# jkulhanek/tetra-nerf

Measured on NVIDIA H100. Metric: rays/sec (4096-ray batch, 300k-tet mesh), higher is better.
Workload: dtype f32 (trace/interp/compositing) + f16w2 tensor-core MLP (fp16 activations x fp16 hi/lo weights, f32 accumulate; per-sample density/colour within 1e-4 of the fp32 oracle, tests/test_gpu_render.py)

## Files before the change

tetra-nerf_b200/csrc/tn_mlp.cuh:

```cuda
#pragma once
#include "tn_common.cuh"
#include "tn_tc.cuh"

namespace tn {

#ifndef TN_MLP_WGS
#define TN_MLP_WGS 3
#endif
constexpr uint32_t MLP_WGS = TN_MLP_WGS;
constexpr uint32_t MLP_THREADS = 128 * MLP_WGS;
constexpr uint32_t MLP_TILE = 64;
constexpr uint32_t MLP_W_BYTES = 32768 + 3 * 65536;
constexpr uint32_t MLP_W_COARSE = 32768 + 2 * 65536;
constexpr uint32_t MLP_OFF_HEAD = MLP_W_BYTES;
constexpr uint32_t MLP_OFF_BARS = MLP_OFF_HEAD + 520 * 4;
constexpr uint32_t MLP_SMEM_BYTES = MLP_OFF_BARS + 8 + 8 * MLP_WGS;
static_assert(MLP_SMEM_BYTES <= 232448, "k_mlp shared memory exceeds 227 KB");
__host__ __device__ constexpr uint32_t mlp_off_layer(int l) { return l == 0 ? 0u : 32768u + 65536u * (uint32_t)(l - 1); }

struct MlpParams {
    const uint32_t *n_active;
    uint32_t S;
    const uint4 *vi;
    const float *bary;
    const float *fshadow;
    const uint8_t *wimg;
    const float *bias;
    const float *head;
    const float *dirbias;
    float *out;
    uint32_t *tile_ctr;
};

constexpr uint32_t MLP_NO_TILE = 0xFFFFFFFFu;

__device__ __forceinline__ float softplus_f(float x) { return x > 20.0f ? x : log1pf(expf(x)); }
__device__ __forceinline__ float sigmoid_f(float x) { return 1.0f / (1.0f + expf(-x)); }

__device__ __forceinline__ float2 ldg_stream2(const float *p) {
    float2 v;
    asm volatile("ld.global.nc.L1::no_allocate.v2.f32 {%0, %1}, [%2];" : "=f"(v.x), "=f"(v.y) : "l"(p));
    return v;
}
__device__ __forceinline__ float4 ldg_stream(const float4 *p) {
    float4 v;
    asm volatile("ld.global.nc.L1::no_allocate.v4.f32 {%0, %1, %2, %3}, [%4];" : "=f"(v.x), "=f"(v.y), "=f"(v.z), "=f"(v.w) : "l"(p));
    return v;
}

__device__ __forceinline__ void wg_sync(uint32_t wg) { asm volatile("bar.sync %0, 128;" ::"r"(1u + wg) : "memory"); }

template <int PREC>
__device__ __forceinline__ void to_operand(float e0, float e1, uint32_t &hi, uint32_t &lo) {
    if (PREC == 2) hi = tc::pack2_f16(e0, e1);
    else tc::split_pack2(e0, e1, hi, lo);
}

template <int PREC>
__device__ __forceinline__ void gather_rows(const uint4 *__restrict__ vi, const float *__restrict__ bary, const float *__restrict__ fshadow, uint64_t row0,
                                            uint64_t total_rows, uint32_t t, uint32_t (&xh)[16], uint32_t (&xl)[16]) {
#pragma unroll
    for (int rr = 0; rr < 2; ++rr) {
        const uint64_t row = row0 + 8u * rr;
        uint4 v = make_uint4(TN_EMPTY, TN_EMPTY, TN_EMPTY, TN_EMPTY);
        float b0 = 0.f, b1 = 0.f, b2 = 0.f;
        if (row < total_rows) {
            v = __ldg(vi + row);
            b0 = __ldg(bary + 3 * row); b1 = __ldg(bary + 3 * row + 1); b2 = __ldg(bary + 3 * row + 2);
        }
        const bool m = v.x != TN_EMPTY;
        const float w0 = __fsub_rn(1.0f, __fadd_rn(__fadd_rn(b0, b1), b2));
        const float *f0 = fshadow + (size_t)v.x * 64 + 2 * t, *f1 = fshadow + (size_t)v.y * 64 + 2 * t;
        const float *f2 = fshadow + (size_t)v.z * 64 + 2 * t, *f3 = fshadow + (size_t)v.w * 64 + 2 * t;
#pragma unroll
        for (int c = 0; c < 8; ++c) {
            float2 o = make_float2(0.f, 0.f);
            if (m) {
                const float2 a0 = ldg_stream2(f0 + 8 * c), a1 = ldg_stream2(f1 + 8 * c), a2 = ldg_stream2(f2 + 8 * c), a3 = ldg_stream2(f3 + 8 * c);
                o.x = __fmaf_rn(b0, a1.x, 0.f); o.y = __fmaf_rn(b0, a1.y, 0.f);
                o.x = __fmaf_rn(b1, a2.x, o.x); o.y = __fmaf_rn(b1, a2.y, o.y);
                o.x = __fmaf_rn(b2, a3.x, o.x); o.y = __fmaf_rn(b2, a3.y, o.y);
                o.x = __fmaf_rn(w0, a0.x, o.x); o.y = __fmaf_rn(w0, a0.y, o.y);
            }
            const int i = 4 * (c >> 1) + 2 * (c & 1) + rr;
            to_operand<PREC>(o.x, o.y, xh[i], xl[i]);
        }
    }
}

template <int PREC, int KSTEPS>
__device__ __forceinline__ void layer_mma(float (&d)[64], const uint32_t (&ah)[4 * KSTEPS], const uint32_t (&al)[4 * KSTEPS], uint32_t w) {
    using namespace tc;
    wgmma_fence();
#pragma unroll
    for (int kk = 0; kk < KSTEPS; ++kk) {
        const uint32_t wb = w + (uint32_t)(kk >> 2) * 32768u + (uint32_t)(kk & 3) * 32u;
        const uint32_t a[4] = {ah[4 * kk], ah[4 * kk + 1], ah[4 * kk + 2], ah[4 * kk + 3]};
        if (PREC == 2) {
            wgmma_rs_f16_n128<0>(d, a, make_desc(wb), kk > 0 ? 1u : 0u);
            wgmma_rs_f16_n128<0>(d, a, make_desc(wb + 16384u), 1u);
        } else {
            const uint32_t b[4] = {al[4 * kk], al[4 * kk + 1], al[4 * kk + 2], al[4 * kk + 3]};
            wgmma_rs_bf16_n128<0>(d, a, make_desc(wb), kk > 0 ? 1u : 0u);
            wgmma_rs_bf16_n128<0>(d, b, make_desc(wb), 1u);
            wgmma_rs_bf16_n128<0>(d, a, make_desc(wb + 16384u), 1u);
        }
    }
    wgmma_commit();
    wgmma_wait0();
    reg_fence(d);
}

template <bool FINE, int PREC>
__global__ void __launch_bounds__(MLP_THREADS, 1) k_mlp(const MlpParams p) {
    using namespace tc;
    extern __shared__ __align__(1024) uint8_t tn_mlp_smem[];
    uint8_t *smem = tn_mlp_smem;
    const float *head_s = reinterpret_cast<const float *>(smem + MLP_OFF_HEAD);
    uint64_t *w_bar = reinterpret_cast<uint64_t *>(smem + MLP_OFF_BARS);
    volatile uint32_t *slots = reinterpret_cast<volatile uint32_t *>(smem + MLP_OFF_BARS + 8);

    constexpr int L = FINE ? 4 : 3;
    constexpr uint32_t WBYTES = FINE ? MLP_W_BYTES : MLP_W_COARSE;
    const uint32_t wg = threadIdx.x >> 7, tid = threadIdx.x & 127u;
    const uint32_t warp = tid >> 5, lane = threadIdx.x & 31u, g = lane >> 2, t = lane & 3u;
    const uint32_t n_active = *p.n_active;
    const uint64_t total_rows = (uint64_t)n_active * p.S;
    const uint32_t ntiles = (uint32_t)((total_rows + MLP_TILE - 1) / MLP_TILE);
    if (blockIdx.x * MLP_WGS >= ntiles) return;

    if (threadIdx.x == 0) {
        mbar_init(w_bar, 1);
        fence_barrier_init();
    }
    for (uint32_t i = threadIdx.x; i < 516; i += MLP_THREADS) const_cast<float *>(head_s)[i] = p.head[i];
    if (tid == 0) {
        const uint32_t first = blockIdx.x * MLP_WGS + wg;
        slots[2 * wg] = first < ntiles ? first : MLP_NO_TILE;
    }
    __syncthreads();
    if (threadIdx.x == 0) {
        mbar_arrive_expect_tx(w_bar, WBYTES);
        for (uint32_t off = 0; off < WBYTES; off += 16384) tma_bulk_g2s(smem + off, p.wimg + off, 16384, w_bar);
    }
    const uint32_t wsm = smem_u32(smem);
    const float *wd = head_s, *wc = head_s + 128;
    bool weights_ready = false;

#pragma unroll 1
    for (uint32_t n = 0;; ++n) {
        wg_sync(wg);
        const uint32_t tile = slots[2 * wg + (n & 1u)];
        if (tile == MLP_NO_TILE) break;
        if (tid == 0) {
            const uint32_t nx = gridDim.x * MLP_WGS + atomicAdd(p.tile_ctr, 1u);
            slots[2 * wg + ((n + 1u) & 1u)] = nx < ntiles ? nx : MLP_NO_TILE;
        }
        const uint64_t row0 = (uint64_t)tile * MLP_TILE + warp * 16u + g, row1 = row0 + 8u;

        uint32_t ah[32], al[32];
        {
            uint32_t xh[16], xl[16];
            gather_rows<PREC>(p.vi, p.bary, p.fshadow, row0, total_rows, t, xh, xl);
            if (!weights_ready) { mbar_wait(w_bar, 0); weights_ready = true; }
            float d[64];
            layer_mma<PREC, 4>(d, xh, xl, wsm + mlp_off_layer(0));
#pragma unroll
            for (int j = 0; j < 16; ++j) {
                const float2 b = __ldg(reinterpret_cast<const float2 *>(p.bias + 8 * j + 2 * t));
                const int i = 4 * (j >> 1) + 2 * (j & 1);
                to_operand<PREC>(fmaxf(d[4 * j] + b.x, 0.f), fmaxf(d[4 * j + 1] + b.y, 0.f), ah[i], al[i]);
                to_operand<PREC>(fmaxf(d[4 * j + 2] + b.x, 0.f), fmaxf(d[4 * j + 3] + b.y, 0.f), ah[i + 1], al[i + 1]);
            }
        }
        float dens0 = 0.f, dens1 = 0.f;
#pragma unroll
        for (int l = 1; l < 3; ++l) {
            float d[64];
            layer_mma<PREC, 8>(d, ah, al, wsm + mlp_off_layer(l));
            const float *bias = p.bias + 128 * l;
#pragma unroll
            for (int j = 0; j < 16; ++j) {
                const int c = 8 * j + 2 * (int)t;
                const float2 b = __ldg(reinterpret_cast<const float2 *>(bias + c));
                const float x0 = fmaxf(d[4 * j] + b.x, 0.f), x1 = fmaxf(d[4 * j + 1] + b.y, 0.f);
                const float y0 = fmaxf(d[4 * j + 2] + b.x, 0.f), y1 = fmaxf(d[4 * j + 3] + b.y, 0.f);
                if (l == 2) {
                    dens0 = fmaf(x0, wd[c], dens0); dens0 = fmaf(x1, wd[c + 1], dens0);
                    dens1 = fmaf(y0, wd[c], dens1); dens1 = fmaf(y1, wd[c + 1], dens1);
                }
                if (l < L - 1) {
                    const int i = 4 * (j >> 1) + 2 * (j & 1);
                    to_operand<PREC>(x0, x1, ah[i], al[i]);
                    to_operand<PREC>(y0, y1, ah[i + 1], al[i + 1]);
                }
            }
        }
        float col0[3] = {0.f, 0.f, 0.f}, col1[3] = {0.f, 0.f, 0.f};
        if (FINE) {
            float d[64];
            layer_mma<PREC, 8>(d, ah, al, wsm + mlp_off_layer(3));
            const float *db0 = p.dirbias + (size_t)((uint32_t)min(row0, total_rows - 1) / p.S) * 128;
            const float *db1 = p.dirbias + (size_t)((uint32_t)min(row1, total_rows - 1) / p.S) * 128;
#pragma unroll
            for (int j = 0; j < 16; ++j) {
                const int c = 8 * j + 2 * (int)t;
                const float2 b0 = __ldg(reinterpret_cast<const float2 *>(db0 + c)), b1 = __ldg(reinterpret_cast<const float2 *>(db1 + c));
                const float x0 = fmaxf(d[4 * j] + b0.x, 0.f), x1 = fmaxf(d[4 * j + 1] + b0.y, 0.f);
                const float y0 = fmaxf(d[4 * j + 2] + b1.x, 0.f), y1 = fmaxf(d[4 * j + 3] + b1.y, 0.f);
#pragma unroll
                for (int ch = 0; ch < 3; ++ch) {
                    const float *w = wc + 128 * ch;
                    col0[ch] = fmaf(x1, w[c + 1], fmaf(x0, w[c], col0[ch]));
                    col1[ch] = fmaf(y1, w[c + 1], fmaf(y0, w[c], col1[ch]));
                }
            }
        }
#pragma unroll
        for (int s = 1; s <= 2; s <<= 1) {
            dens0 += __shfl_xor_sync(0xffffffffu, dens0, s);
            dens1 += __shfl_xor_sync(0xffffffffu, dens1, s);
            if (FINE) {
#pragma unroll
                for (int ch = 0; ch < 3; ++ch) {
                    col0[ch] += __shfl_xor_sync(0xffffffffu, col0[ch], s);
                    col1[ch] += __shfl_xor_sync(0xffffffffu, col1[ch], s);
                }
            }
        }
        if (t < 2) {
            const uint64_t row = t == 0 ? row0 : row1;
            const float dn = t == 0 ? dens0 : dens1;
            if (row < total_rows) {
                const float sigma = softplus_f(dn + head_s[512]);
                if (FINE) {
                    const float c0 = t == 0 ? col0[0] : col1[0], c1 = t == 0 ? col0[1] : col1[1], c2 = t == 0 ? col0[2] : col1[2];
                    reinterpret_cast<float4 *>(p.out)[row] =
                        make_float4(sigma, sigmoid_f(c0 + head_s[513]), sigmoid_f(c1 + head_s[514]), sigmoid_f(c2 + head_s[515]));
                } else {
                    p.out[row] = sigma;
                }
            }
        }
    }
    if (!weights_ready) mbar_wait(w_bar, 0);
}

}
```

tetra-nerf_b200/csrc/tn_mlp_bwd.cuh:

```cuda
#pragma once
#include <type_traits>

#include "tn_common.cuh"
#include "tn_mlp.cuh"
#include "tn_tc.cuh"

namespace tn {

constexpr uint32_t BWD_THREADS = 128;
constexpr uint32_t BWD_TILE = 64;
constexpr uint32_t BWD_STAGE = 32768;
constexpr uint32_t BWD_OFF_RING = 0;
constexpr uint32_t BWD_OFF_X = 65536;
constexpr uint32_t BWD_OFF_H = 81920;
constexpr uint32_t BWD_OFF_DA = BWD_OFF_H + 3 * 32768;
constexpr uint32_t BWD_OFF_HEAD = BWD_OFF_DA + 32768;
constexpr uint32_t BWD_OFF_SUMS = BWD_OFF_HEAD + 2048;
constexpr uint32_t BWD_OFF_BARS = BWD_OFF_SUMS + 7 * 512;
constexpr uint32_t BWD_SMEM_BYTES = BWD_OFF_BARS + 32;
static_assert(BWD_SMEM_BYTES <= 232448, "k_mlp_bwd shared memory exceeds 227 KB");
static_assert(BWD_OFF_X % 1024 == 0 && BWD_OFF_H % 1024 == 0 && BWD_OFF_DA % 1024 == 0, "swizzled operands need 1024-byte alignment");
constexpr uint32_t BWD_WIMG_BYTES = 7 * BWD_STAGE;
constexpr uint32_t BWD_NSEQ = 14;

struct MlpBwdParams {
    const uint32_t *n_active;
    uint32_t S;
    const uint4 *vi;
    const float *bary;
    const float *fshadow;
    const uint8_t *wimg;
    const float *bias;
    const float *head;
    const float *dirbias;
    const float4 *dout;
    float *gshadow;
    float *gw;
    float *g_dirbias;
    uint32_t *tile_ctr;
};
struct MlpBwdDetParams : MlpBwdParams {
    float *part;
    float *gdb_part;
    float *dx;
};
template <bool DET>
using MlpBwdParamsT = typename std::conditional<DET, MlpBwdDetParams, MlpBwdParams>::type;
constexpr uint32_t GW_W1 = 0, GW_W2 = 8192, GW_W3 = 24576, GW_W4B = 40960, GW_B1 = 57344, GW_B2 = 57472, GW_B3 = 57600, GW_WD = 57728, GW_WC = 57856,
                   GW_SUMS = 58240 , GW_W4DIR = 58244 , GW_B4 = 61700, GW_TOTAL = 61828;

constexpr uint32_t BWD_PARTS = 256;
constexpr uint32_t BWD_PART_STRIDE = GW_SUMS;
constexpr uint32_t BWD_DET_OFF_BARS = BWD_OFF_SUMS + 4 * 7 * 512;
constexpr uint32_t BWD_DET_SMEM_BYTES = BWD_DET_OFF_BARS + 32;
static_assert(BWD_DET_SMEM_BYTES <= 232448, "k_mlp_bwd<true> shared memory exceeds 227 KB");
__host__ __device__ __forceinline__ uint32_t bwd_part_lo(uint32_t q, uint32_t ntiles) { return (uint32_t)(((uint64_t)q * ntiles) / BWD_PARTS); }
__host__ __device__ __forceinline__ uint32_t bwd_part_of(uint32_t tile, uint32_t ntiles) {
    return (uint32_t)((((uint64_t)tile + 1) * BWD_PARTS - 1) / ntiles);
}
__device__ __forceinline__ uint32_t bwd_det_first(uint32_t q, uint32_t step, uint32_t ntiles) {
    for (; q < BWD_PARTS; q += step)
        if (bwd_part_lo(q, ntiles) < bwd_part_lo(q + 1, ntiles)) return bwd_part_lo(q, ntiles);
    return MLP_NO_TILE;
}

__device__ __forceinline__ void red_add_v2(float *dst, float a, float b) {
    asm volatile("red.global.add.v2.f32 [%0], {%1, %2};" ::"l"(dst), "f"(a), "f"(b) : "memory");
}
__device__ __forceinline__ void red_add_v4(float *dst, float a, float b, float c, float d) {
    asm volatile("red.global.add.v4.f32 [%0], {%1, %2, %3, %4};" ::"l"(dst), "f"(a), "f"(b), "f"(c), "f"(d) : "memory");
}
__device__ __forceinline__ float4 quad_of_row(float2 p0, float2 p1, uint32_t t) {
    const bool odd = (t & 1u) != 0u;
    const float2 send = odd ? p0 : p1;
    float2 recv;
    recv.x = __shfl_xor_sync(0xffffffffu, send.x, 1);
    recv.y = __shfl_xor_sync(0xffffffffu, send.y, 1);
    return odd ? make_float4(recv.x, recv.y, p1.x, p1.y) : make_float4(p0.x, p0.y, recv.x, recv.y);
}

__device__ __forceinline__ void st_pair(uint32_t base, uint32_t R, uint32_t j, uint32_t t, uint32_t lo_off, uint32_t h, uint32_t l) {
    const uint32_t rowoff = (R >> 3) * 1024u + (R & 7u) * 128u + 4u * t;
    asm volatile(
        "{\n\t.reg .b32 a, x, y;\n\t"
        "and.b32 x, %2, 7;\n\txor.b32 x, x, %3;\n\tshl.b32 x, x, 4;\n\t"
        "shr.b32 y, %2, 3;\n\tshl.b32 y, y, 13;\n\t"
        "add.u32 a, %0, %1;\n\tadd.u32 a, a, x;\n\tadd.u32 a, a, y;\n\t"
        "st.shared.b32 [a], %5;\n\tadd.u32 a, a, %4;\n\tst.shared.b32 [a], %6;\n\t}" ::"r"(base),
        "r"(rowoff), "r"(j), "r"(R & 7u), "r"(lo_off), "r"(h), "r"(l)
        : "memory");
}

template <bool DET = false>
__device__ __forceinline__ void colsum2(float *dst, uint32_t c, float s0, float s1, uint32_t lane, uint32_t warp = 0) {
#pragma unroll
    for (int m = 4; m <= 16; m <<= 1) {
        s0 += __shfl_xor_sync(0xffffffffu, s0, m);
        s1 += __shfl_xor_sync(0xffffffffu, s1, m);
    }
    if constexpr (DET) {
        if (lane < 4) { float *w = dst + warp * (7u * 128u); w[c] += s0; w[c + 1] += s1; }
    } else {
        if (lane < 4) { atomicAdd(dst + c, s0); atomicAdd(dst + c + 1, s1); }
    }
}

template <int NB, bool DET = false>
__device__ __forceinline__ void dw_half(uint32_t sDA, uint32_t sHb, uint32_t h_lo_off, uint32_t mh, float *dst, uint32_t warp, uint32_t g, uint32_t t,
                                        bool first = false) {
    using namespace tc;
    float d[32 * NB];
#pragma unroll
    for (int i = 0; i < 32 * NB; ++i) d[i] = 0.f;
    wgmma_fence();
#pragma unroll
    for (int term = 0; term < 3; ++term) {
        const uint32_t ao = term == 1 ? 16384u : 0u, bo = term == 2 ? h_lo_off : 0u;
#pragma unroll
        for (uint32_t kk = 0; kk < 4; ++kk) {
            const uint64_t da = make_desc(sDA + ao + mh * 8192u + kk * 2048u, 8192u, 1024u);
            const uint64_t db = make_desc(sHb + bo + kk * 2048u, 8192u, 1024u);
            if constexpr (NB == 2) wgmma_ss_bf16_n128<1, 1>(d, da, db, 1u);
            else wgmma_ss_bf16_n64<1, 1>(d, da, db, 1u);
        }
    }
    wgmma_commit();
    wgmma_wait0();
    reg_fence(d);
    const uint32_t o = mh * 64u + warp * 16u + g + 8u * (t & 1u);
#pragma unroll
    for (int j = 0; j < 4 * NB * 2; ++j) {
        const float4 q = quad_of_row(make_float2(d[4 * j], d[4 * j + 1]), make_float2(d[4 * j + 2], d[4 * j + 3]), t);
        if constexpr (DET) {
            float4 *a = reinterpret_cast<float4 *>(dst + (size_t)o * (64u * NB) + 8u * j + 4u * (t >> 1));
            float4 r = q;
            if (!first) { const float4 b = *a; r = make_float4(b.x + q.x, b.y + q.y, b.z + q.z, b.w + q.w); }
            *a = r;
        } else {
            red_add_v4(dst + (size_t)o * (64u * NB) + 8u * j + 4u * (t >> 1), q.x, q.y, q.z, q.w);
        }
    }
}

template <int N>
__device__ __forceinline__ void zero(float (&d)[N]) {
#pragma unroll
    for (int i = 0; i < N; ++i) d[i] = 0.f;
}

__device__ __forceinline__ void frag_pair(float x0, float x1, float y0, float y1, int j, uint32_t (&ah)[32], uint32_t (&al)[32]) {
    const int i = 4 * (j >> 1) + 2 * (j & 1);
    tc::split_pack2(x0, x1, ah[i], al[i]);
    tc::split_pack2(y0, y1, ah[i + 1], al[i + 1]);
}

template <bool DET>
__global__ void __launch_bounds__(BWD_THREADS, 1) k_mlp_bwd(const MlpBwdParamsT<DET> p) {
    using namespace tc;
    extern __shared__ __align__(1024) uint8_t tn_bwd_smem[];
    constexpr uint32_t OFF_BARS = DET ? BWD_DET_OFF_BARS : BWD_OFF_BARS;
    uint8_t *smem = tn_bwd_smem;
    float *head_s = reinterpret_cast<float *>(smem + BWD_OFF_HEAD);
    float *sums = reinterpret_cast<float *>(smem + BWD_OFF_SUMS);
    uint64_t *ring_full = reinterpret_cast<uint64_t *>(smem + OFF_BARS);
    volatile uint32_t *slots = reinterpret_cast<volatile uint32_t *>(smem + OFF_BARS + 16);

    const uint32_t tid = threadIdx.x, warp = tid >> 5, lane = tid & 31u, g = lane >> 2, t = lane & 3u;
    const uint32_t n_active = *p.n_active;
    const uint64_t total_rows = (uint64_t)n_active * p.S;
    const uint32_t ntiles = (uint32_t)((total_rows + BWD_TILE - 1) / BWD_TILE);
    uint32_t first_tile = blockIdx.x;
    if constexpr (DET) {
        if (ntiles == 0) return;
        first_tile = bwd_det_first(blockIdx.x, gridDim.x, ntiles);
        if (first_tile == MLP_NO_TILE) return;
    } else {
        if (blockIdx.x >= ntiles) return;
    }

    if (tid == 0) {
        mbar_init(&ring_full[0], 1); mbar_init(&ring_full[1], 1);
        fence_barrier_init();
        slots[0] = first_tile;
    }
    for (uint32_t i = tid; i < 512; i += BWD_THREADS) head_s[i] = p.head[i];
    for (uint32_t i = tid; i < (DET ? 4u : 1u) * 7 * 128; i += BWD_THREADS) sums[i] = 0.f;
    __syncthreads();
    const uint32_t sR = smem_u32(smem + BWD_OFF_RING), sX = smem_u32(smem + BWD_OFF_X), sH = smem_u32(smem + BWD_OFF_H), sDA = smem_u32(smem + BWD_OFF_DA);
    const float *wd = head_s, *wc = head_s + 128;

    auto ring_issue = [&](uint32_t i) {
        const uint32_t q = i % BWD_NSEQ;
        const uint32_t img = q < 7u ? q : (q == 13u ? 0u : (q & 1u ? 12u - q : 14u - q));
        uint64_t *bar = &ring_full[i & 1u];
        mbar_arrive_expect_tx(bar, BWD_STAGE);
        tma_bulk_g2s(smem + BWD_OFF_RING + (i & 1u) * BWD_STAGE, p.wimg + img * BWD_STAGE, 16384, bar);
        tma_bulk_g2s(smem + BWD_OFF_RING + (i & 1u) * BWD_STAGE + 16384u, p.wimg + img * BWD_STAGE + 16384u, 16384, bar);
    };
    if (tid == 0) ring_issue(0);
    uint32_t seq = 0;
    auto ring_acquire = [&](bool more) -> uint32_t {
        wg_sync(0);
        if (tid == 0 && more) ring_issue(seq + 1u);
        mbar_wait(&ring_full[seq & 1u], (seq >> 1) & 1u);
        const uint32_t w = sR + (seq & 1u) * BWD_STAGE;
        ++seq;
        return w;
    };
    auto publish = [&]() {
        fence_proxy_async();
        wg_sync(0);
    };

#pragma unroll 1
    for (uint32_t n = 0;; ++n) {
        wg_sync(0);
        const uint32_t tile = slots[n & 1u];
        if (tile == MLP_NO_TILE) break;
        uint32_t part_q = 0;
        bool part_first = false, part_last = false;
        if constexpr (DET) {
            part_q = bwd_part_of(tile, ntiles);
            part_first = tile == bwd_part_lo(part_q, ntiles);
            part_last = tile + 1u == bwd_part_lo(part_q + 1u, ntiles);
        }
        float *gw = p.gw;
        if constexpr (DET) gw = p.part + (size_t)part_q * BWD_PART_STRIDE;
        if (tid == 0) {
            if constexpr (DET) {
                slots[(n + 1u) & 1u] = part_last ? bwd_det_first(part_q + gridDim.x, gridDim.x, ntiles) : tile + 1u;
            } else {
                const uint32_t nx = gridDim.x + atomicAdd(p.tile_ctr, 1u);
                slots[(n + 1u) & 1u] = nx < ntiles ? nx : MLP_NO_TILE;
            }
        }
        const uint32_t R0 = warp * 16u + g, R1 = R0 + 8u;
        const uint64_t row0 = (uint64_t)tile * BWD_TILE + R0, row1 = row0 + 8u;
        const bool valid0 = row0 < total_rows, valid1 = row1 < total_rows;
        const float4 z4 = make_float4(0.f, 0.f, 0.f, 0.f);
        const float4 g0 = valid0 ? __ldg(p.dout + row0) : z4, g1 = valid1 ? __ldg(p.dout + row1) : z4;

        uint32_t ah[32], al[32];
        unsigned long long mask[3];
        float d[64];
        const bool more_tiles = slots[(n + 1u) & 1u] != MLP_NO_TILE;
        {
            uint32_t xh[16], xl[16];
            gather_rows<3>(p.vi, p.bary, p.fshadow, row0, total_rows, t, xh, xl);
#pragma unroll
            for (int c = 0; c < 8; ++c) {
                const int i = 4 * (c >> 1) + 2 * (c & 1);
                st_pair(sX, R0, (uint32_t)c, t, 8192u, xh[i], xl[i]);
                st_pair(sX, R1, (uint32_t)c, t, 8192u, xh[i + 1], xl[i + 1]);
            }
            const uint32_t w = ring_acquire(true);
            zero(d);
            wgmma_fence();
#pragma unroll
            for (int kk = 0; kk < 4; ++kk) {
                const uint32_t a[4] = {xh[4 * kk], xh[4 * kk + 1], xh[4 * kk + 2], xh[4 * kk + 3]};
                const uint32_t b[4] = {xl[4 * kk], xl[4 * kk + 1], xl[4 * kk + 2], xl[4 * kk + 3]};
                wgmma_rs_bf16_n128<0>(d, a, make_desc(w + kk * 32u), kk > 0 ? 1u : 0u);
                wgmma_rs_bf16_n128<0>(d, b, make_desc(w + kk * 32u), 1u);
                wgmma_rs_bf16_n128<0>(d, a, make_desc(w + 16384u + kk * 32u), 1u);
            }
            wgmma_commit();
            wgmma_wait0();
            reg_fence(d);
        }
#pragma unroll
        for (int l = 0; l < 3; ++l) {
            if (l > 0) {
                uint32_t w = ring_acquire(true);
                zero(d);
                wgmma_fence();
#pragma unroll
                for (int kk = 0; kk < 8; ++kk) {
                    const uint32_t a[4] = {ah[4 * kk], ah[4 * kk + 1], ah[4 * kk + 2], ah[4 * kk + 3]};
                    const uint32_t b[4] = {al[4 * kk], al[4 * kk + 1], al[4 * kk + 2], al[4 * kk + 3]};
                    const uint32_t wo = (uint32_t)(kk >> 2) * 16384u + (uint32_t)(kk & 3) * 32u;
                    wgmma_rs_bf16_n128<0>(d, a, make_desc(w + wo), kk > 0 ? 1u : 0u);
                    wgmma_rs_bf16_n128<0>(d, b, make_desc(w + wo), 1u);
                }
                wgmma_commit();
                wgmma_wait0();
                w = ring_acquire(true);
                wgmma_fence();
#pragma unroll
                for (int kk = 0; kk < 8; ++kk) {
                    const uint32_t a[4] = {ah[4 * kk], ah[4 * kk + 1], ah[4 * kk + 2], ah[4 * kk + 3]};
                    wgmma_rs_bf16_n128<0>(d, a, make_desc(w + (uint32_t)(kk >> 2) * 16384u + (uint32_t)(kk & 3) * 32u), 1u);
                }
                wgmma_commit();
                wgmma_wait0();
                reg_fence(d);
            }
            const float *bias = p.bias + 128 * l;
            const uint32_t hb = sH + 32768u * l;
            unsigned long long mk = 0ull;
#pragma unroll
            for (int j = 0; j < 16; ++j) {
                const uint32_t c = 8u * j + 2u * t;
                const float2 b = __ldg(reinterpret_cast<const float2 *>(bias + c));
                const float v0 = d[4 * j] + b.x, v1 = d[4 * j + 1] + b.y, v2 = d[4 * j + 2] + b.x, v3 = d[4 * j + 3] + b.y;
                mk |= (unsigned long long)((v0 > 0.f ? 1u : 0u) | (v1 > 0.f ? 2u : 0u) | (v2 > 0.f ? 4u : 0u) | (v3 > 0.f ? 8u : 0u)) << (4 * j);
                const float x0 = fmaxf(v0, 0.f), x1 = fmaxf(v1, 0.f), y0 = fmaxf(v2, 0.f), y1 = fmaxf(v3, 0.f);
                frag_pair(x0, x1, y0, y1, j, ah, al);
                const int i = 4 * (j >> 1) + 2 * (j & 1);
                st_pair(hb, R0, (uint32_t)j, t, 16384u, ah[i], al[i]);
                st_pair(hb, R1, (uint32_t)j, t, 16384u, ah[i + 1], al[i + 1]);
                if (l == 2)
                    colsum2<DET>(sums + 3 * 128, c, g0.x * x0 + g1.x * y0, g0.x * x1 + g1.x * y1, lane, warp);
            }
            mask[l] = mk;
        }
        {
            uint32_t w = ring_acquire(true);
            zero(d);
            wgmma_fence();
#pragma unroll
            for (int kk = 0; kk < 8; ++kk) {
                const uint32_t a[4] = {ah[4 * kk], ah[4 * kk + 1], ah[4 * kk + 2], ah[4 * kk + 3]};
                const uint32_t b[4] = {al[4 * kk], al[4 * kk + 1], al[4 * kk + 2], al[4 * kk + 3]};
                const uint32_t wo = (uint32_t)(kk >> 2) * 16384u + (uint32_t)(kk & 3) * 32u;
                wgmma_rs_bf16_n128<0>(d, a, make_desc(w + wo), kk > 0 ? 1u : 0u);
                wgmma_rs_bf16_n128<0>(d, b, make_desc(w + wo), 1u);
            }
            wgmma_commit();
            wgmma_wait0();
            w = ring_acquire(true);
            wgmma_fence();
#pragma unroll
            for (int kk = 0; kk < 8; ++kk) {
                const uint32_t a[4] = {ah[4 * kk], ah[4 * kk + 1], ah[4 * kk + 2], ah[4 * kk + 3]};
                wgmma_rs_bf16_n128<0>(d, a, make_desc(w + (uint32_t)(kk >> 2) * 16384u + (uint32_t)(kk & 3) * 32u), 1u);
            }
            wgmma_commit();
            wgmma_wait0();
            reg_fence(d);
            const uint32_t ray0 = (uint32_t)(min(row0, total_rows - 1) / p.S), ray1 = (uint32_t)(min(row1, total_rows - 1) / p.S);
            const float *db0 = p.dirbias + (size_t)ray0 * 128, *db1 = p.dirbias + (size_t)ray1 * 128;
#pragma unroll
            for (int j = 0; j < 16; ++j) {
                const uint32_t c = 8u * j + 2u * t;
                const float2 b0 = __ldg(reinterpret_cast<const float2 *>(db0 + c)), b1 = __ldg(reinterpret_cast<const float2 *>(db1 + c));
                const float v0 = d[4 * j] + b0.x, v1 = d[4 * j + 1] + b0.y, v2 = d[4 * j + 2] + b1.x, v3 = d[4 * j + 3] + b1.y;
                const float x0 = fmaxf(v0, 0.f), x1 = fmaxf(v1, 0.f), y0 = fmaxf(v2, 0.f), y1 = fmaxf(v3, 0.f);
                colsum2<DET>(sums + 4 * 128, c, g0.y * x0 + g1.y * y0, g0.y * x1 + g1.y * y1, lane, warp);
                colsum2<DET>(sums + 5 * 128, c, g0.z * x0 + g1.z * y0, g0.z * x1 + g1.z * y1, lane, warp);
                colsum2<DET>(sums + 6 * 128, c, g0.w * x0 + g1.w * y0, g0.w * x1 + g1.w * y1, lane, warp);
                const float wa0 = wc[c], wa1 = wc[c + 1], wb0 = wc[128 + c], wb1 = wc[128 + c + 1], wc0 = wc[256 + c], wc1 = wc[256 + c + 1];
                d[4 * j] = v0 > 0.f ? fmaf(g0.w, wc0, fmaf(g0.z, wb0, g0.y * wa0)) : 0.f;
                d[4 * j + 1] = v1 > 0.f ? fmaf(g0.w, wc1, fmaf(g0.z, wb1, g0.y * wa1)) : 0.f;
                d[4 * j + 2] = v2 > 0.f ? fmaf(g1.w, wc0, fmaf(g1.z, wb0, g1.y * wa0)) : 0.f;
                d[4 * j + 3] = v3 > 0.f ? fmaf(g1.w, wc1, fmaf(g1.z, wb1, g1.y * wa1)) : 0.f;
                frag_pair(d[4 * j], d[4 * j + 1], d[4 * j + 2], d[4 * j + 3], j, ah, al);
                const int i = 4 * (j >> 1) + 2 * (j & 1);
                st_pair(sDA, R0, (uint32_t)j, t, 16384u, ah[i], al[i]);
                st_pair(sDA, R1, (uint32_t)j, t, 16384u, ah[i + 1], al[i + 1]);
            }
            const uint32_t ray_lo = __shfl_sync(0xffffffffu, ray0, 0), ray_hi = __shfl_sync(0xffffffffu, ray1, 28);
#pragma unroll 1
            for (uint32_t sl = ray_lo; sl <= ray_hi; ++sl) {
                const bool in0 = valid0 && ray0 == sl, in1 = valid1 && ray1 == sl;
#pragma unroll
                for (int j = 0; j < 16; ++j) {
                    float s0 = (in0 ? d[4 * j] : 0.f) + (in1 ? d[4 * j + 2] : 0.f);
                    float s1 = (in0 ? d[4 * j + 1] : 0.f) + (in1 ? d[4 * j + 3] : 0.f);
#pragma unroll
                    for (int m = 4; m <= 16; m <<= 1) {
                        s0 += __shfl_xor_sync(0xffffffffu, s0, m);
                        s1 += __shfl_xor_sync(0xffffffffu, s1, m);
                    }
                    if constexpr (DET) {
                        if (lane < 4) *reinterpret_cast<float2 *>(p.gdb_part + (4 * ((size_t)tile + sl) + warp) * 128 + 8u * j + 2u * t) = make_float2(s0, s1);
                    } else {
                        if (lane < 4) red_add_v2(p.g_dirbias + (size_t)sl * 128 + 8u * j + 2u * t, s0, s1);
                    }
                }
            }
            publish();
        }
#pragma unroll 1
        for (int l = 2; l >= 0; --l) {
            float *gdst = gw + (l == 2 ? GW_W4B : (l == 1 ? GW_W3 : GW_W2));
            const uint32_t hb = sH + 32768u * (uint32_t)l;
            dw_half<2, DET>(sDA, hb, 16384u, 0, gdst, warp, g, t, part_first);
            dw_half<2, DET>(sDA, hb, 16384u, 1, gdst, warp, g, t, part_first);
            uint32_t w = ring_acquire(true);
            zero(d);
            wgmma_fence();
#pragma unroll
            for (int kk = 0; kk < 8; ++kk) {
                const uint32_t a[4] = {ah[4 * kk], ah[4 * kk + 1], ah[4 * kk + 2], ah[4 * kk + 3]};
                const uint32_t b[4] = {al[4 * kk], al[4 * kk + 1], al[4 * kk + 2], al[4 * kk + 3]};
                wgmma_rs_bf16_n128<1>(d, a, make_desc(w + kk * 2048u, 16384u, 1024u), kk > 0 ? 1u : 0u);
                wgmma_rs_bf16_n128<1>(d, b, make_desc(w + kk * 2048u, 16384u, 1024u), 1u);
            }
            wgmma_commit();
            wgmma_wait0();
            w = ring_acquire(true);
            wgmma_fence();
#pragma unroll
            for (int kk = 0; kk < 8; ++kk) {
                const uint32_t a[4] = {ah[4 * kk], ah[4 * kk + 1], ah[4 * kk + 2], ah[4 * kk + 3]};
                wgmma_rs_bf16_n128<1>(d, a, make_desc(w + kk * 2048u, 16384u, 1024u), 1u);
            }
            wgmma_commit();
            wgmma_wait0();
            reg_fence(d);
            const unsigned long long mk = l == 2 ? mask[2] : (l == 1 ? mask[1] : mask[0]);
            float *bsum = sums + 128 * l;
#pragma unroll
            for (int j = 0; j < 16; ++j) {
                const uint32_t c = 8u * j + 2u * t;
                float e0 = d[4 * j], e1 = d[4 * j + 1], e2 = d[4 * j + 2], e3 = d[4 * j + 3];
                if (l == 2) {
                    e0 = fmaf(g0.x, wd[c], e0); e1 = fmaf(g0.x, wd[c + 1], e1);
                    e2 = fmaf(g1.x, wd[c], e2); e3 = fmaf(g1.x, wd[c + 1], e3);
                }
                const uint32_t m = (uint32_t)(mk >> (4 * j)) & 15u;
                e0 = (m & 1u) ? e0 : 0.f; e1 = (m & 2u) ? e1 : 0.f; e2 = (m & 4u) ? e2 : 0.f; e3 = (m & 8u) ? e3 : 0.f;
                colsum2<DET>(bsum, c, e0 + e2, e1 + e3, lane, warp);
                frag_pair(e0, e1, e2, e3, j, ah, al);
                const int i = 4 * (j >> 1) + 2 * (j & 1);
                st_pair(sDA, R0, (uint32_t)j, t, 16384u, ah[i], al[i]);
                st_pair(sDA, R1, (uint32_t)j, t, 16384u, ah[i + 1], al[i + 1]);
            }
            publish();
        }
        dw_half<1, DET>(sDA, sX, 8192u, 0, gw + GW_W1, warp, g, t, part_first);
        dw_half<1, DET>(sDA, sX, 8192u, 1, gw + GW_W1, warp, g, t, part_first);
        {
            const uint32_t w = ring_acquire(more_tiles);
            float dx[32];
            zero(dx);
            wgmma_fence();
#pragma unroll
            for (int kk = 0; kk < 8; ++kk) {
                const uint32_t a[4] = {ah[4 * kk], ah[4 * kk + 1], ah[4 * kk + 2], ah[4 * kk + 3]};
                const uint32_t b[4] = {al[4 * kk], al[4 * kk + 1], al[4 * kk + 2], al[4 * kk + 3]};
                wgmma_rs_bf16_n64<1>(dx, a, make_desc(w + kk * 2048u, 16384u, 1024u), kk > 0 ? 1u : 0u);
                wgmma_rs_bf16_n64<1>(dx, b, make_desc(w + kk * 2048u, 16384u, 1024u), 1u);
                wgmma_rs_bf16_n64<1>(dx, a, make_desc(w + 16384u + kk * 2048u, 16384u, 1024u), 1u);
            }
            wgmma_commit();
            wgmma_wait0();
            reg_fence(dx);
            float4 q[8];
#pragma unroll
            for (int j = 0; j < 8; ++j) q[j] = quad_of_row(make_float2(dx[4 * j], dx[4 * j + 1]), make_float2(dx[4 * j + 2], dx[4 * j + 3]), t);
            const uint64_t row = (t & 1u) ? row1 : row0;
            if constexpr (DET) {
                if (row < total_rows) {
                    float4 *dst = reinterpret_cast<float4 *>(p.dx + row * 64 + 4u * (t >> 1));
#pragma unroll
                    for (int j = 0; j < 8; ++j) dst[2 * j] = q[j];
                }
            } else if (row < total_rows) {
                const uint4 v = __ldg(p.vi + row);
                if (v.x != TN_EMPTY) {
                    const float b0 = __ldg(p.bary + 3 * row), b1 = __ldg(p.bary + 3 * row + 1), b2 = __ldg(p.bary + 3 * row + 2);
                    const float w0 = 1.0f - ((b0 + b1) + b2);
                    const uint32_t vs[4] = {v.x, v.y, v.z, v.w};
                    const float ws[4] = {w0, b0, b1, b2};
#pragma unroll
                    for (int k = 0; k < 4; ++k) {
                        float *dst = p.gshadow + (size_t)vs[k] * 64 + 4u * (t >> 1);
#pragma unroll
                        for (int j = 0; j < 8; ++j) red_add_v4(dst + 8 * j, ws[k] * q[j].x, ws[k] * q[j].y, ws[k] * q[j].z, ws[k] * q[j].w);
                    }
                }
            }
        }
        if constexpr (DET) {
            if (part_last) {
                const uint32_t c = tid;
#pragma unroll 1
                for (uint32_t k = 0; k < 7; ++k) {
                    float *s = sums + k * 128 + c;
                    gw[GW_B1 + k * 128 + c] = ((s[0] + s[896]) + s[1792]) + s[2688];
                    s[0] = 0.f; s[896] = 0.f; s[1792] = 0.f; s[2688] = 0.f;
                }
            }
        }
    }
    if constexpr (DET) return;
    __syncthreads();
    for (uint32_t c = tid; c < 128; c += BWD_THREADS) {
        atomicAdd(p.gw + GW_B1 + c, sums[c]);
        atomicAdd(p.gw + GW_B2 + c, sums[128 + c]);
        atomicAdd(p.gw + GW_B3 + c, sums[256 + c]);
        atomicAdd(p.gw + GW_WD + c, sums[384 + c]);
        atomicAdd(p.gw + GW_WC + c, sums[512 + c]);
        atomicAdd(p.gw + GW_WC + 128 + c, sums[640 + c]);
        atomicAdd(p.gw + GW_WC + 256 + c, sums[768 + c]);
    }
}

}
```

Measured before the change: 3.319 million.

## Batch feature gathers and prefetch next tile's indices in MLP kernel

Splits the gather into an index/barycentric load and a feature gather that issues all 64 feature loads per thread up front, before any FMA, so more memory requests are in flight at once. Empty rows now load from vertex 0 instead of being predicated off. The tile scheduler draws one tile ahead, so the next tile's vi/bary rows and the current tile's dirbias rows can be L1-prefetched while the MLP runs. The cost is many more live registers (64 float2 values), which may spill or lower occupancy, plus the extra redundant loads for empty rows.

```diff
diff --git a/tetra-nerf_b200/csrc/tn_mlp.cuh b/tetra-nerf_b200/csrc/tn_mlp.cuh
--- a/tetra-nerf_b200/csrc/tn_mlp.cuh
+++ b/tetra-nerf_b200/csrc/tn_mlp.cuh
@@ -56,32 +56,64 @@
     else tc::split_pack2(e0, e1, hi, lo);
 }
 
+struct GatherRows {
+    uint4 v[2];
+    float b[2][3];
+};
+__device__ __forceinline__ GatherRows load_gather_rows(const uint4 *__restrict__ vi, const float *__restrict__ bary, uint64_t row0, uint64_t total_rows) {
+    GatherRows r;
+#pragma unroll
+    for (int rr = 0; rr < 2; ++rr) {
+        const uint64_t row = row0 + 8u * rr;
+        r.v[rr] = make_uint4(TN_EMPTY, TN_EMPTY, TN_EMPTY, TN_EMPTY);
+        r.b[rr][0] = r.b[rr][1] = r.b[rr][2] = 0.f;
+        if (row < total_rows) {
+            r.v[rr] = __ldg(vi + row);
+            r.b[rr][0] = __ldg(bary + 3 * row); r.b[rr][1] = __ldg(bary + 3 * row + 1); r.b[rr][2] = __ldg(bary + 3 * row + 2);
+        }
+    }
+    return r;
+}
+__device__ __forceinline__ void prefetch_l1(const void *p) { asm volatile("prefetch.global.L1 [%0];" ::"l"(p)); }
+__device__ __forceinline__ void prefetch_gather_rows(const uint4 *vi, const float *bary, uint64_t row0, uint64_t total_rows) {
+#pragma unroll
+    for (int rr = 0; rr < 2; ++rr) {
+        const uint64_t row = row0 + 8u * rr;
+        if (row < total_rows) {
+            prefetch_l1(vi + row);
+            prefetch_l1(bary + 3 * row);
+        }
+    }
+}
+
 template <int PREC>
-__device__ __forceinline__ void gather_rows(const uint4 *__restrict__ vi, const float *__restrict__ bary, const float *__restrict__ fshadow, uint64_t row0,
-                                            uint64_t total_rows, uint32_t t, uint32_t (&xh)[16], uint32_t (&xl)[16]) {
-#pragma unroll
-    for (int rr = 0; rr < 2; ++rr) {
-        const uint64_t row = row0 + 8u * rr;
-        uint4 v = make_uint4(TN_EMPTY, TN_EMPTY, TN_EMPTY, TN_EMPTY);
-        float b0 = 0.f, b1 = 0.f, b2 = 0.f;
-        if (row < total_rows) {
-            v = __ldg(vi + row);
-            b0 = __ldg(bary + 3 * row); b1 = __ldg(bary + 3 * row + 1); b2 = __ldg(bary + 3 * row + 2);
-        }
-        const bool m = v.x != TN_EMPTY;
+__device__ __forceinline__ void gather_rows(const GatherRows &r, const float *__restrict__ fshadow, uint32_t t, uint32_t (&xh)[16], uint32_t (&xl)[16]) {
+    float2 a[2][4][8];
+#pragma unroll
+    for (int rr = 0; rr < 2; ++rr) {
+        const uint4 v = r.v[rr].x != TN_EMPTY ? r.v[rr] : make_uint4(0u, 0u, 0u, 0u);
+        const uint32_t vs[4] = {v.x, v.y, v.z, v.w};
+#pragma unroll
+        for (int k = 0; k < 4; ++k) {
+            const float *f = fshadow + (size_t)vs[k] * 64 + 2 * t;
+#pragma unroll
+            for (int c = 0; c < 8; ++c) a[rr][k][c] = ldg_stream2(f + 8 * c);
+        }
+    }
+#pragma unroll
+    for (int rr = 0; rr < 2; ++rr) {
+        const bool m = r.v[rr].x != TN_EMPTY;
+        const float b0 = r.b[rr][0], b1 = r.b[rr][1], b2 = r.b[rr][2];
         const float w0 = __fsub_rn(1.0f, __fadd_rn(__fadd_rn(b0, b1), b2));
-        const float *f0 = fshadow + (size_t)v.x * 64 + 2 * t, *f1 = fshadow + (size_t)v.y * 64 + 2 * t;
-        const float *f2 = fshadow + (size_t)v.z * 64 + 2 * t, *f3 = fshadow + (size_t)v.w * 64 + 2 * t;
 #pragma unroll
         for (int c = 0; c < 8; ++c) {
-            float2 o = make_float2(0.f, 0.f);
-            if (m) {
-                const float2 a0 = ldg_stream2(f0 + 8 * c), a1 = ldg_stream2(f1 + 8 * c), a2 = ldg_stream2(f2 + 8 * c), a3 = ldg_stream2(f3 + 8 * c);
-                o.x = __fmaf_rn(b0, a1.x, 0.f); o.y = __fmaf_rn(b0, a1.y, 0.f);
-                o.x = __fmaf_rn(b1, a2.x, o.x); o.y = __fmaf_rn(b1, a2.y, o.y);
-                o.x = __fmaf_rn(b2, a3.x, o.x); o.y = __fmaf_rn(b2, a3.y, o.y);
-                o.x = __fmaf_rn(w0, a0.x, o.x); o.y = __fmaf_rn(w0, a0.y, o.y);
-            }
+            const float2 a0 = a[rr][0][c], a1 = a[rr][1][c], a2 = a[rr][2][c], a3 = a[rr][3][c];
+            float2 o;
+            o.x = __fmaf_rn(b0, a1.x, 0.f); o.y = __fmaf_rn(b0, a1.y, 0.f);
+            o.x = __fmaf_rn(b1, a2.x, o.x); o.y = __fmaf_rn(b1, a2.y, o.y);
+            o.x = __fmaf_rn(b2, a3.x, o.x); o.y = __fmaf_rn(b2, a3.y, o.y);
+            o.x = __fmaf_rn(w0, a0.x, o.x); o.y = __fmaf_rn(w0, a0.y, o.y);
+            if (!m) o = make_float2(0.f, 0.f);
             const int i = 4 * (c >> 1) + 2 * (c & 1) + rr;
             to_operand<PREC>(o.x, o.y, xh[i], xl[i]);
         }
@@ -134,9 +166,14 @@
         fence_barrier_init();
     }
     for (uint32_t i = threadIdx.x; i < 516; i += MLP_THREADS) const_cast<float *>(head_s)[i] = p.head[i];
+    auto draw = [&]() {
+        const uint32_t nx = gridDim.x * MLP_WGS + atomicAdd(p.tile_ctr, 1u);
+        return nx < ntiles ? nx : MLP_NO_TILE;
+    };
     if (tid == 0) {
         const uint32_t first = blockIdx.x * MLP_WGS + wg;
         slots[2 * wg] = first < ntiles ? first : MLP_NO_TILE;
+        slots[2 * wg + 1] = draw();
     }
     __syncthreads();
     if (threadIdx.x == 0) {
@@ -146,22 +183,29 @@
     const uint32_t wsm = smem_u32(smem);
     const float *wd = head_s, *wc = head_s + 128;
     bool weights_ready = false;
+    const uint32_t lrow = warp * 16u + g;
+    uint32_t tile = slots[2 * wg];
 
 #pragma unroll 1
     for (uint32_t n = 0;; ++n) {
         wg_sync(wg);
-        const uint32_t tile = slots[2 * wg + (n & 1u)];
         if (tile == MLP_NO_TILE) break;
-        if (tid == 0) {
-            const uint32_t nx = gridDim.x * MLP_WGS + atomicAdd(p.tile_ctr, 1u);
-            slots[2 * wg + ((n + 1u) & 1u)] = nx < ntiles ? nx : MLP_NO_TILE;
-        }
-        const uint64_t row0 = (uint64_t)tile * MLP_TILE + warp * 16u + g, row1 = row0 + 8u;
+        const uint32_t next = slots[2 * wg + ((n + 1u) & 1u)];
+        if (tid == 0) slots[2 * wg + (n & 1u)] = draw();
+        const uint64_t row0 = (uint64_t)tile * MLP_TILE + lrow, row1 = row0 + 8u;
+        const float *db0 = nullptr, *db1 = nullptr;
 
         uint32_t ah[32], al[32];
         {
             uint32_t xh[16], xl[16];
-            gather_rows<PREC>(p.vi, p.bary, p.fshadow, row0, total_rows, t, xh, xl);
+            gather_rows<PREC>(load_gather_rows(p.vi, p.bary, row0, total_rows), p.fshadow, t, xh, xl);
+            if (next != MLP_NO_TILE) prefetch_gather_rows(p.vi, p.bary, (uint64_t)next * MLP_TILE + lrow, total_rows);
+            if (FINE) {
+                db0 = p.dirbias + (size_t)((uint32_t)min(row0, total_rows - 1) / p.S) * 128;
+                db1 = p.dirbias + (size_t)((uint32_t)min(row1, total_rows - 1) / p.S) * 128;
+                prefetch_l1(db0 + 32 * t);
+                prefetch_l1(db1 + 32 * t);
+            }
             if (!weights_ready) { mbar_wait(w_bar, 0); weights_ready = true; }
             float d[64];
             layer_mma<PREC, 4>(d, xh, xl, wsm + mlp_off_layer(0));
@@ -200,8 +244,6 @@
         if (FINE) {
             float d[64];
             layer_mma<PREC, 8>(d, ah, al, wsm + mlp_off_layer(3));
-            const float *db0 = p.dirbias + (size_t)((uint32_t)min(row0, total_rows - 1) / p.S) * 128;
-            const float *db1 = p.dirbias + (size_t)((uint32_t)min(row1, total_rows - 1) / p.S) * 128;
 #pragma unroll
             for (int j = 0; j < 16; ++j) {
                 const int c = 8 * j + 2 * (int)t;
@@ -242,6 +284,7 @@
                 }
             }
         }
+        tile = next;
     }
     if (!weights_ready) mbar_wait(w_bar, 0);
 }
diff --git a/tetra-nerf_b200/csrc/tn_mlp_bwd.cuh b/tetra-nerf_b200/csrc/tn_mlp_bwd.cuh
--- a/tetra-nerf_b200/csrc/tn_mlp_bwd.cuh
+++ b/tetra-nerf_b200/csrc/tn_mlp_bwd.cuh
@@ -246,7 +246,7 @@
         const bool more_tiles = slots[(n + 1u) & 1u] != MLP_NO_TILE;
         {
             uint32_t xh[16], xl[16];
-            gather_rows<3>(p.vi, p.bary, p.fshadow, row0, total_rows, t, xh, xl);
+            gather_rows<3>(load_gather_rows(p.vi, p.bary, row0, total_rows), p.fshadow, t, xh, xl);
 #pragma unroll
             for (int c = 0; c < 8; ++c) {
                 const int i = 4 * (c >> 1) + 2 * (c & 1);
```

Result: faster. 3.552 million (median of 6 runs) (+7.0%).
